# NVIDIA/MinkowskiEngine

Hardware: AMD Instinct MI355X
Metric: MinkowskiConvolution fwd+bwd Mpoints/sec (100k-pt 3D, k=3) (higher is better)
Workload: dtype f32

## Files before the change

minkowskiengine_amd/_lib.py:

```python
import ctypes
import os

_HERE = os.path.dirname(os.path.abspath(__file__))
_TAG = os.environ.get("ME_AMD_LIB_TAG", "")
LIB_PATH = os.path.join(_HERE, f"libme_amd_{_TAG}.so" if _TAG else "libme_amd.so")

ME_MAX_DIM = 7
ME_MAX_TILE_ROWS = 256
ME_GROUP_ROWS = 16
ME_MAX_BATCH_GROUPS = 4

c_i32, c_i64, c_vp = ctypes.c_int32, ctypes.c_int64, ctypes.c_void_p


class MeRegion(ctypes.Structure):
    _fields_ = [
        ("ncol", c_i32),
        ("region_type", c_i32),
        ("kernel_size", c_i32 * ME_MAX_DIM),
        ("dilation", c_i32 * ME_MAX_DIM),
        ("tensor_stride", c_i32 * ME_MAX_DIM),
        ("n_offsets", c_i32),
        ("offsets_dev", c_vp),
    ]
# ... 241 lines not shown
    "me_direct_max_pool_f32": (ctypes.c_int, [c_vp, c_i32, c_vp, c_vp, c_i32, c_i64, c_i64, c_i64, c_i32, c_vp, c_vp, c_vp, c_i64, c_vp]),
    "me_direct_max_pool_bf16": (ctypes.c_int, [c_vp, c_i32, c_vp, c_vp, c_i32, c_i64, c_i64, c_i64, c_i32, c_vp, c_vp, c_vp, c_i64, c_vp]),
    "me_direct_max_pool_f64": (ctypes.c_int, [c_vp, c_i32, c_vp, c_vp, c_i32, c_i64, c_i64, c_i64, c_i32, c_vp, c_vp, c_vp, c_i64, c_vp]),
    "me_direct_max_pool_backward_workspace_bytes": (c_i64, [c_i64, c_i32]),
    "me_direct_max_pool_backward_f32": (ctypes.c_int, [c_vp, c_vp, c_i32, c_i64, c_i32, c_i64, c_vp, c_vp, c_i64, c_vp]),
    "me_direct_max_pool_backward_bf16": (ctypes.c_int, [c_vp, c_vp, c_i32, c_i64, c_i32, c_i64, c_vp, c_vp, c_i64, c_vp]),
    "me_direct_max_pool_backward_f64": (ctypes.c_int, [c_vp, c_vp, c_i32, c_i64, c_i32, c_i64, c_vp, c_vp, c_i64, c_vp]),
    "me_union_tables": (ctypes.c_int, [c_vp, c_i64, c_vp, c_i64, c_i64, c_vp, c_vp, c_vp, c_vp, c_vp]),
    "me_union_arith_f32": (ctypes.c_int, [c_vp, c_vp, c_i32, c_vp, c_vp, c_i64, c_i64, c_i64, c_i32, c_vp, c_vp]),
    "me_union_arith_bf16": (ctypes.c_int, [c_vp, c_vp, c_i32, c_vp, c_vp, c_i64, c_i64, c_i64, c_i32, c_vp, c_vp]),
    "me_union_arith_f64": (ctypes.c_int, [c_vp, c_vp, c_i32, c_vp, c_vp, c_i64, c_i64, c_i64, c_i32, c_vp, c_vp]),
    "me_union_arith_backward_f32": (ctypes.c_int, [c_vp, c_vp, c_vp, c_i32, c_vp, c_vp, c_vp, c_vp, c_i64, c_i64, c_i64, c_i32, c_vp, c_vp, c_vp]),
    "me_union_arith_backward_bf16": (ctypes.c_int, [c_vp, c_vp, c_vp, c_i32, c_vp, c_vp, c_vp, c_vp, c_i64, c_i64, c_i64, c_i32, c_vp, c_vp, c_vp]),
    "me_union_arith_backward_f64": (ctypes.c_int, [c_vp, c_vp, c_vp, c_i32, c_vp, c_vp, c_vp, c_vp, c_i64, c_i64, c_i64, c_i32, c_vp, c_vp, c_vp]),
    "me_csr_from_coo_workspace_bytes": (c_i64, [c_i64]),
    "me_csr_from_coo": (ctypes.c_int, [c_vp, c_vp, c_vp, c_i32, c_i64, c_i64, c_vp, c_vp, c_vp, c_vp, c_i64, c_vp]),
    "me_csr_gather_f32": (ctypes.c_int, [c_vp, c_i32, c_vp, c_vp, c_vp, c_vp, c_i64, c_vp, c_vp]),
    "me_csr_gather_bf16": (ctypes.c_int, [c_vp, c_i32, c_vp, c_vp, c_vp, c_vp, c_i64, c_vp, c_vp]),
    "me_csr_gather_f64": (ctypes.c_int, [c_vp, c_i32, c_vp, c_vp, c_vp, c_vp, c_i64, c_vp, c_vp]),
    "me_conv_forward_naive_f32": (ctypes.c_int, [c_vp, c_i32, c_vp, c_i32, c_vp, c_vp, c_vp, c_i64, c_i64,
                                                 c_vp, c_vp]),
    "me_conv_backward_naive_f32": (ctypes.c_int, [c_vp, c_i32, c_vp, c_i32, c_vp, c_vp, c_vp, c_vp, c_i64,
                                                  c_i64, c_vp, c_vp, c_vp]),
}

DEBUG_SIGNATURES = {
    "me_debug_variants_compiled": (c_i32, []),
    "me_debug_set_conv_variant": (ctypes.c_int, [ctypes.c_int]),
    "me_debug_conv_timing": (ctypes.c_int, [c_vp, c_i32]),
    "me_debug_conv_timing_f32x3": (ctypes.c_int, [c_vp, c_i32]),
    "me_debug_set_wgrad_config": (None, [ctypes.c_int, ctypes.c_int]),
    "me_debug_set_wgrad_order": (None, [ctypes.c_int]),
    "me_debug_set_dgrad_reduce_tail": (None, [ctypes.c_int]),
    "me_debug_set_wgrad_ws": (None, [ctypes.c_int]),
    "me_debug_set_tile_dispatch": (None, [ctypes.c_int]),
    "me_debug_set_wgrad_mb": (None, [ctypes.c_int]),
    "me_debug_set_bf16_shape": (None, [ctypes.c_int, ctypes.c_int]),
    "me_debug_set_bf16_deep": (None, [ctypes.c_int]),
    "me_debug_set_bf16_twobuf": (None, [ctypes.c_int]),
    "me_debug_set_f32_fused_split": (None, [ctypes.c_int]),
    "me_debug_set_bf16_ws": (None, [ctypes.c_int]),
    "me_debug_set_halo": (None, [ctypes.c_int, ctypes.c_int, ctypes.c_int, ctypes.c_int]),
    "me_debug_halo_mode": (c_i32, []),
    "me_debug_set_stem": (None, [ctypes.c_int, ctypes.c_int]),
    "me_debug_set_stem_tiles_per_wg": (None, [ctypes.c_int]),
    "me_debug_halo_timing": (ctypes.c_int, [c_vp, c_i32]),
    "me_debug_set_bf16_ws_fuse": (None, [ctypes.c_int]),
    "me_debug_set_bf16_ws_depth": (None, [ctypes.c_int]),
    "me_debug_set_bf16_ws_ncw": (None, [ctypes.c_int]),
    "me_debug_set_rowwise_groups": (None, [ctypes.c_int]),
    "me_debug_set_rowwise_items_per_wg": (None, [ctypes.c_int]),
    "me_debug_set_insert_fused": (None, [ctypes.c_int]),
    "me_debug_ws_timing": (ctypes.c_int, [c_vp, c_i32]),
    "me_debug_set_bf16_offsync": (None, [ctypes.c_int]),
    "me_debug_set_bf16_splitk": (None, [ctypes.c_int]),
    "me_debug_set_bf16_splitk_mode": (None, [ctypes.c_int]),
    "me_debug_bf16_timing": (ctypes.c_int, [c_vp, c_i32]),
}

_lib = None


def load():
    global _lib
    if _lib is not None:
        return _lib
# ... 72 lines not shown
```

minkowskiengine_amd/csrc/conv_f32x3.hip:

```cpp
#include <type_traits>
#include <vector>
#include "conv_common.hpp"
#include "conv_ws.hpp"
#include "wgrad_reduce.hpp"

namespace me {


__host__ __device__ constexpr int x3_group_shares(int nc) { return nc >= 96 ? 1 : (nc == 64 ? 2 : 4); }

__host__ __device__ constexpr int conv_f32x3_lds_bytes(int nc, int kc, int tile_rows) {
  return (tile_rows + 1) * (nc + kAccPad) * 4 + 2 * ME_MAX_BATCH_GROUPS * 16 * (3 * x3_stage_ld(kc) * 2 + 4);
}

template <int KC>
__global__ __launch_bounds__(256) void k_pack_weights_f32x3(const float *__restrict__ w, int c_src, int c_dst,
                                                           int transposed, int nchunks, int ncb,
                                                           u32x4 *__restrict__ wp, int64_t total) {
  constexpr int KS = KC / 32;
  const int64_t e = (int64_t)blockIdx.x * blockDim.x + threadIdx.x;
  if (e >= total) return;
  const int lane = (int)(e % 64);
  int64_t r = e / 64;
  const int v = (int)(r % KS);
  r /= KS;
  const int cb = (int)(r % ncb);
  r /= ncb;
  const int c = (int)(r % nchunks);
  const int64_t k = r / nchunks;
  const int q = lane >> 4, i16 = lane & 15;
  const int col = cb * 16 + i16;
  float val[8];
#pragma unroll
  for (int j = 0; j < 8; ++j) {
    const int ch = c * KC + v * 32 + q * 8 + j;
    val[j] = 0.f;
    if (ch < c_src && col < c_dst) {
      const int64_t idx = transposed ? (k * c_dst + col) * c_src + ch : (k * c_src + ch) * c_dst + col;
      val[j] = w[idx];
    }
  }
  u32x4 p1, p2, p3;
  split3<true>(f32x4{val[0], val[1], val[2], val[3]}, f32x4{val[4], val[5], val[6], val[7]}, p1, p2, p3);
  const int64_t base = ((((k * nchunks + c) * ncb + cb) * 3) * KS + v) * 64 + lane;
  wp[base] = p1;
// ... 312 lines not shown
#pragma unroll
    for (int j = 0; j < ORD; ++j)
      if (j * NT + tid < tile_rows) s_ord[j * NT + tid] = my_ord[j];
    __syncthreads();
  }
  for (int x = tid; x < tile_rows * NC / 4; x += NT) {
    const int row = x / (NC / 4);
    const int c4 = x % (NC / 4);
    const int cc = col_base + c4 * 4;
    if (row < rows_here && cc < c_dst) {
      const f32x4 v = *reinterpret_cast<const f32x4 *>(&s_acc[row * ACC_LD + c4 * 4]);
      const int64_t grow = order ? (int64_t)s_ord[row] : row0 + row;
      float *o = dst + grow * c_dst + cc;
      if (vec_out) {
        *reinterpret_cast<f32x4 *>(o) = v;
      } else {
        o[0] = v.x;
        if (cc + 1 < c_dst) o[1] = v.y;
        if (cc + 2 < c_dst) o[2] = v.z;
        if (cc + 3 < c_dst) o[3] = v.w;
      }
    }
  }
  if (TIMED) {
    tick(6);
    if (tid == 0) {
#pragma unroll
      for (int t = 0; t < 7; ++t) atomicAdd(&d_x3_timing[t], tm[t]);
      atomicAdd(&d_x3_timing[7], (unsigned long long)n_it);
    }
  }
}

template <typename T>
__device__ __forceinline__ const T &only_arg(const T &t) { return t; }

template <int NC, int KC, bool EXACT, bool SMALL, bool TIMED = false, int PRIO = 2, int ABL = 0, int NCW = 4,
          bool TAIL = false, typename... TAIL_ARG>
__global__ __launch_bounds__((NCW + 4) * 64, 1) void k_conv_tile_f32x3_ws(
    const float *__restrict__ src, int c_src, const bf16x8 *__restrict__ wp, int c_dst,
    const int32_t *__restrict__ plan_src, const int32_t *__restrict__ plan_dst,
    const int32_t *__restrict__ batch_desc, const int32_t *__restrict__ tile_bptr,
    const int32_t *__restrict__ order, float *__restrict__ dst, int64_t n_tgt, int tile_rows, int batch_groups,
    TAIL_ARG... tail) {
  static_assert(sizeof...(TAIL_ARG) == (TAIL ? 1 : 0), "TAIL: exactly one WgTail argument");
  typedef int i32x2 __attribute__((ext_vector_type(2)));
  typedef StageLayout<KC> SL;
  static_assert(NC == 64 || NC == 128, "multiplier waves of 16 or 32 columns");
  static_assert(NCW == 4 || (NCW == 8 && NC == 128), "four multiplier waves, or eight on a 128-column slab");
  constexpr int CB = NC / (16 * NCW);
  constexpr int NTP = 256;
  constexpr int NT = NCW * 64 + NTP;
  constexpr int LD = SL::kLd;
  constexpr int ACC_LD = NC + kAccPad;
  constexpr int KS = KC / 32;
  constexpr int F8 = KC / 8;
  constexpr int CAP = ME_MAX_BATCH_GROUPS * 16;
  constexpr int ITER = (CAP * F8 + NTP - 1) / NTP;
  constexpr int PLANE = CAP * LD;
  (void)batch_groups;

  extern __shared__ __attribute__((aligned(16))) char smem[];
  unsigned n_tiles = gridDim.x;
  if constexpr (TAIL) {
    const WgTail &t = only_arg(tail...);
    n_tiles = (unsigned)t.n_tiles;
    if (blockIdx.x >= n_tiles) {
      if (blockIdx.y + 1 == gridDim.y) wgrad_reduce_tail<NT>(t.r, t.nb, (int)(blockIdx.x - n_tiles), smem);
      return;
    }
  }
  float *s_acc = reinterpret_cast<float *>(smem);
  __bf16 *s_a = reinterpret_cast<__bf16 *>(s_acc + (tile_rows + 1) * ACC_LD);
  int32_t *s_dst = reinterpret_cast<int32_t *>(s_a + 2 * 3 * PLANE);

  const int tid = threadIdx.x;
  const int lane = tid & 63;
  const int wave = __builtin_amdgcn_readfirstlane(tid >> 6);
  const int i16 = lane & 15;
  const int q = lane >> 4;
  const int tile = tile_bptr[n_tiles + 1 + blockIdx.x];
  const int col_base = blockIdx.y * NC;
  const int nchunks = (c_src + KC - 1) / KC;
  const int ncb = (c_dst + 15) / 16;

  for (int x = tid; x < (tile_rows + 1) * ACC_LD / 4; x += NT)
    reinterpret_cast<f32x4 *>(s_acc)[x] = f32x4{0.f, 0.f, 0.f, 0.f};
  constexpr int ORD = (ME_MAX_TILE_ROWS + NT - 1) / NT;
  int32_t my_ord[ORD];
#pragma unroll
  for (int j = 0; j < ORD; ++j) {
    const int r = j * NT + tid;
    my_ord[j] = (order != nullptr && r < tile_rows && (int64_t)tile * tile_rows + r < n_tgt)
                    ? order[(int64_t)tile * tile_rows + r] : 0;
  }

  const int b0 = tile_bptr[tile];
  const int nb = tile_bptr[tile + 1] - b0;
  const int n_it = nb * nchunks;
  struct Desc {
    int chunk, g0, ng, k;
  };
  auto locate = [&](int it) {
    int r = min(it, n_it - 1);
    Desc d;
    d.chunk = 0;
    while (r >= nb) {
      r -= nb;
      ++d.chunk;
    }
    const i32x2 v = *reinterpret_cast<const i32x2 *>(batch_desc + 2 * (int64_t)(b0 + r));
    d.g0 = v.x;
    d.ng = v.y & 255;
    d.k = (int)((uint32_t)v.y >> 8);
    return d;
  };

  if (n_it > 0 && wave >= NCW) {
    const int ptid = tid - NCW * 64;
    f32x4 stage[2][ITER][2];
    int32_t dstv[2] = {tile_rows, tile_rows};
    int32_t sidx[2][ITER];
    auto load_sidx = [&](const Desc &d, int32_t (&sx)[ITER]) {
      const char *pb = reinterpret_cast<const char *>(plan_src + (int64_t)d.g0 * 16);
#pragma unroll
      for (int j = 0; j < ITER; ++j)
        sx[j] = *reinterpret_cast<const int32_t *>(pb + (unsigned)(min((j * NTP + ptid) / F8, CAP - 1) * 4));
    };
    const char *srcb = reinterpret_cast<const char *>(src);
    const unsigned row_bytes = (unsigned)c_src * 4u;
    auto gather = [&](const Desc &d, const int32_t (&sx)[ITER], f32x4 (&st)[ITER][2], int32_t &dv) {
      const int c0 = d.chunk * KC;
      dv = *reinterpret_cast<const int32_t *>(reinterpret_cast<const char *>(plan_dst + (int64_t)d.g0 * 16) +
                                             (unsigned)(min(ptid, CAP - 1) * 4));
#pragma unroll
      for (int j = 0; j < ITER; ++j) {
        const int ch = c0 + ((j * NTP + ptid) % F8) * 8;
        const int chl = EXACT ? ch : min(ch, c_src - 8);
        const int sr = max(sx[j], 0);
        const f32x4 *p;
        if (SMALL) p = reinterpret_cast<const f32x4 *>(srcb + (__umul24((unsigned)sr, row_bytes) + (unsigned)chl * 4u));
        else p = reinterpret_cast<const f32x4 *>(src + (int64_t)sr * c_src + chl);
        st[j][0] = p[0];
        st[j][1] = p[1];
      }
    };
    auto write_stage = [&](const Desc &d, const f32x4 (&st)[ITER][2], int32_t dv, int buf) {
      const int c0 = d.chunk * KC;
// ... 38 lines not shown
    auto produce = [&](const Desc &dx, const Desc &dx2, const Desc &dx3, int buf, f32x4 (&st)[ITER][2], int32_t &dv,
                       int32_t (&sx_nx)[ITER], int32_t (&sx_cu)[ITER]) {
      if (ABL != 6) write_stage(dx, st, dv, buf);
      load_sidx(dx3, sx_cu);
      if (ABL != 5 || !started) gather(dx2, sx_nx, st, dv);
    };
    Desc dA = locate(0), dB = locate(1), dC = locate(2), dD = locate(3), dE = locate(4);
    load_sidx(dA, sidx[0]);
    load_sidx(dB, sidx[1]);
    gather(dA, sidx[0], stage[0], dstv[0]);
    gather(dB, sidx[1], stage[1], dstv[1]);
    load_sidx(dC, sidx[0]);
    produce(dA, dC, dD, 0, stage[0], dstv[0], sidx[0], sidx[1]);
    started = true;
    __syncthreads();
    unsigned long long tm_a = 0, tm_b = 0, t_prev = TIMED ? __builtin_amdgcn_s_memtime() : 0ull;
    auto iteration = [&](int it, int P, f32x4 (&st_nx)[ITER][2], int32_t &dv_nx, int32_t (&sx_nx)[ITER],
                         int32_t (&sx_cu)[ITER]) {
      produce(dB, dD, dE, P ^ 1, st_nx, dv_nx, sx_nx, sx_cu);
      if (TIMED) {
        asm volatile("s_waitcnt lgkmcnt(0)" ::: "memory");
        const unsigned long long now = __builtin_amdgcn_s_memtime();
        tm_a += now - t_prev;
        t_prev = now;
      }
      __syncthreads();
      if (TIMED) {
        const unsigned long long now = __builtin_amdgcn_s_memtime();
        tm_b += now - t_prev;
        t_prev = now;
      }
      dA = dB; dB = dC; dC = dD; dD = dE;
      dE = locate(it + 5);
    };
    int it = 0;
    for (; it + 1 < n_it; it += 2) {
      iteration(it, 0, stage[1], dstv[1], sidx[1], sidx[0]);
      iteration(it + 1, 1, stage[0], dstv[0], sidx[0], sidx[1]);
    }
    if (it < n_it) iteration(it, 0, stage[1], dstv[1], sidx[1], sidx[0]);
    if (TIMED && tid == NCW * 64) {
      atomicAdd(&d_x3_timing[1], tm_a);
      atomicAdd(&d_x3_timing[2], tm_b);
    }
  } else if (n_it > 0) {
    __builtin_amdgcn_s_setprio(PRIO);
    const int cbi0 = col_base / 16 + wave * CB;
    bf16x8 w[2][CB][3][KS];
    auto load_w = [&](const Desc &d, bf16x8 (&wd)[CB][3][KS]) {
#pragma unroll
      for (int c = 0; c < CB; ++c) {
        const bf16x8 *p = wp + (((((int64_t)d.k * nchunks + d.chunk) * ncb + min(cbi0 + c, ncb - 1)) * 3) * KS) * 64 + lane;
#pragma unroll
        for (int pl = 0; pl < 3; ++pl) {
#pragma unroll
          for (int v = 0; v < KS; ++v) wd[c][pl][v] = p[(pl * KS + v) * 64];
        }
      }
    };
    int pofs[KS];
#pragma unroll
    for (int sx = 0; sx < KS; ++sx) pofs[sx] = ((sx * 4 + q) ^ SL::swz(i16)) * 8;
    auto multiply = [&](const Desc &d, const bf16x8 (&wc)[CB][3][KS], int buf, auto &&next_w) {
      const __bf16 *rowp = s_a + buf * 3 * PLANE + i16 * LD;
      const int32_t *dstp = s_dst + buf * CAP + i16;
      float *accp = &s_acc[wave * CB * 16 + q * 4];
      if (d.ng >= 4) consume_batch_ws<2, 2, CB, KC, 3, ABL>(rowp, pofs, wc, dstp, accp, ACC_LD, next_w);
      else if (d.ng == 3) consume_batch_ws<2, 1, CB, KC, 3, ABL>(rowp, pofs, wc, dstp, accp, ACC_LD, next_w);
      else if (d.ng == 2) consume_batch_ws<2, 0, CB, KC, 3, ABL>(rowp, pofs, wc, dstp, accp, ACC_LD, next_w);
      else consume_batch_ws<1, 0, CB, KC, 3, ABL>(rowp, pofs, wc, dstp, accp, ACC_LD, next_w);
    };
    Desc dA = locate(0), dB = locate(1);
    load_w(dA, w[0]);
    __syncthreads();
    unsigned long long tm_a = 0, tm_b = 0, t_prev = TIMED ? __builtin_amdgcn_s_memtime() : 0ull;
    auto iteration = [&](int it, int P, bf16x8 (&w_cu)[CB][3][KS], bf16x8 (&w_nx)[CB][3][KS]) {
      multiply(dA, w_cu, P, [&]() {
        if (ABL != 4 || it == 0) load_w(dB, w_nx);
      });
      if (TIMED) {
        asm volatile("s_waitcnt lgkmcnt(0)" ::: "memory");
        const unsigned long long now = __builtin_amdgcn_s_memtime();
        tm_a += now - t_prev;
        t_prev = now;
      }
      __syncthreads();
      if (TIMED) {
        const unsigned long long now = __builtin_amdgcn_s_memtime();
        tm_b += now - t_prev;
        t_prev = now;
      }
      dA = dB;
      dB = locate(it + 2);
    };
    int it = 0;
    for (; it + 1 < n_it; it += 2) {
      iteration(it, 0, w[0], w[1]);
      iteration(it + 1, 1, w[1], w[0]);
    }
    if (it < n_it) iteration(it, 0, w[0], w[1]);
    if (TIMED && tid == 0) {
      atomicAdd(&d_x3_timing[4], tm_a);
      atomicAdd(&d_x3_timing[0], tm_b);
      atomicAdd(&d_x3_timing[7], (unsigned long long)n_it);
    }
  } else {
    __syncthreads();
  }

  const int64_t row0 = (int64_t)tile * tile_rows;
  const int rows_here = (int)min((int64_t)tile_rows, n_tgt - row0);
  const bool vec_out = (c_dst % 4) == 0;
  int32_t *s_ord = reinterpret_cast<int32_t *>(s_a);
  if (order != nullptr) {
#pragma unroll
    for (int j = 0; j < ORD; ++j)
      if (j * NT + tid < tile_rows) s_ord[j * NT + tid] = my_ord[j];
    __syncthreads();
  }
  for (int x = tid; x < tile_rows * NC / 4; x += NT) {
    const int row = x / (NC / 4);
    const int c4 = x % (NC / 4);
    const int cc = col_base + c4 * 4;
    if (row < rows_here && cc < c_dst) {
      const f32x4 v = *reinterpret_cast<const f32x4 *>(&s_acc[row * ACC_LD + c4 * 4]);
      const int64_t grow = order ? (int64_t)s_ord[row] : row0 + row;
      float *o = dst + grow * c_dst + cc;
      if (vec_out) {
        *reinterpret_cast<f32x4 *>(o) = v;
      } else {
        o[0] = v.x;
        if (cc + 1 < c_dst) o[1] = v.y;
        if (cc + 2 < c_dst) o[2] = v.z;
        if (cc + 3 < c_dst) o[3] = v.w;
      }
    }
  }
}


#ifdef ME_DEBUG_VARIANTS
__device__ __forceinline__ unsigned ring_addr(const int32_t *p) {
  typedef __attribute__((address_space(3))) const char lds_char;
  return (unsigned)(uintptr_t)(lds_char *)p;
}
__device__ __forceinline__ void ring_wait(unsigned flag_addr, int target) {
  for (;;) {
    int v;
    asm volatile("ds_read_b32 %0, %1\n\ts_waitcnt lgkmcnt(0)" : "=v"(v) : "v"(flag_addr) : "memory");
    if (__builtin_amdgcn_readfirstlane(v) >= target) break;
    __builtin_amdgcn_s_sleep(1);
  }
}
__device__ __forceinline__ void ring_signal(unsigned flag_addr, int lane) {
  if (lane == 0) asm volatile("ds_add_u32 %0, %1" : : "v"(flag_addr), "v"(1) : "memory");
}

__host__ __device__ constexpr int conv_f32x3_ring_lds_bytes(int nc, int kc, int tile_rows, int ns) {
  return (tile_rows + 1) * (nc + kAccPad) * 4 + ns * ME_MAX_BATCH_GROUPS * 16 * (3 * x3_stage_ld(kc) * 2 + 4) + 64;
}

template <int NC, int KC, bool EXACT, bool SMALL, int NCW, int NS>
__global__ __launch_bounds__((NCW + 4) * 64, 1) void k_conv_tile_f32x3_ring(
    const float *__restrict__ src, int c_src, const bf16x8 *__restrict__ wp, int c_dst,
    const int32_t *__restrict__ plan_src, const int32_t *__restrict__ plan_dst,
    const int32_t *__restrict__ batch_desc, const int32_t *__restrict__ tile_bptr,
    const int32_t *__restrict__ order, float *__restrict__ dst, int64_t n_tgt, int tile_rows, int batch_groups) {
  typedef int i32x2 __attribute__((ext_vector_type(2)));
  typedef StageLayout<KC> SL;
// ... 578 lines not shown
        ++round;
      }
    };
    for (;;) {
      iteration(w[0], w[1]);
      if (end) break;
      iteration(w[1], w[0]);
      if (end) break;
    }
  }
}

#endif

extern int g_conv_variant;

struct ConvVariantX3 {
  int nc, slabs, kc;
};

static ConvVariantX3 conv_variant_f32x3(int c_src, int c_dst) {
  ConvVariantX3 v;
  if (c_dst % 128 == 0) v.nc = 128;
  else if (c_dst % 96 == 0) v.nc = 96;
  else v.nc = c_dst <= 32 ? 32 : 64;
  v.slabs = (int)ceil_div(c_dst, v.nc);
  if (c_src % 128 == 0 && v.nc <= 64) v.kc = 128;
  else if (c_src % 64 == 0) v.kc = 64;
  else if (c_src % 96 == 0) v.kc = 96;
  else v.kc = c_src <= 32 ? 32 : 64;
  return v;
}

template <int NC, int KC>
static int launch_conv_tile_f32x3(const float *src, int c_src, const bf16x8 *wp, int c_dst, int slabs,
                                  const int32_t *plan_src, const int32_t *plan_dst, const int32_t *batch_desc,
                                  const int32_t *tile_bptr, const int32_t *order, float *dst, int64_t n_tgt,
                                  int tile_rows, int batch_groups, hipStream_t stream, bool small,
                                  const WgTail *tail = nullptr) {
  int lds = conv_f32x3_lds_bytes(NC, KC, tile_rows);
  ME_CHECK(lds <= kLdsBudget, "tile_rows too large for the LDS of one workgroup");
  const bool exact = (c_src % KC) == 0;
  const bool fast = small && exact;
  typedef void (*kernel_t)(const float *, int, const bf16x8 *, int, const int32_t *, const int32_t *, const int32_t *,
                           const int32_t *, const int32_t *, float *, int64_t, int, int);
#ifdef ME_DEBUG_VARIANTS
  constexpr bool kHasPingPong = true;
#else
  constexpr bool kHasPingPong = !(NC == 64 || NC == 128);
#endif
  kernel_t fn = nullptr;
  if constexpr (kHasPingPong)
    fn = fast ? &k_conv_tile_f32x3<NC, KC, true, true> : &k_conv_tile_f32x3<NC, KC, false, false>;
  if constexpr (NC == 64 || NC == 128) {
#ifdef ME_DEBUG_VARIANTS
    if constexpr (KC == 64 || KC == 128) {
      if (small && exact && (g_conv_variant == 40 || g_conv_variant == 41)) {
        constexpr int RNCW = NC == 128 ? 8 : 4;
        constexpr bool kHas3 = KC == 64;
        const bool three = kHas3 && g_conv_variant != 41 && conv_f32x3_ring_lds_bytes(NC, KC, tile_rows, 3) <= kLdsBudget;
        kernel_t rk = &k_conv_tile_f32x3_ring<NC, KC, true, true, RNCW, 2>;
        if constexpr (kHas3) {
          if (three) rk = &k_conv_tile_f32x3_ring<NC, KC, true, true, RNCW, 3>;
        }
        const int rlds = conv_f32x3_ring_lds_bytes(NC, KC, tile_rows, three ? 3 : 2);
        ME_CHECK(rlds <= kLdsBudget, "tile_rows too large for the LDS of one workgroup (ring kernel)");
        static bool ring_attr[2] = {false, false};
        if (rlds > 48 * 1024 && !ring_attr[three ? 1 : 0]) {
          ME_HIP(hipFuncSetAttribute(reinterpret_cast<const void *>(rk), hipFuncAttributeMaxDynamicSharedMemorySize,
                                     kLdsBudget));
          ring_attr[three ? 1 : 0] = true;
        }
        const dim3 rgrid((unsigned)ceil_div(n_tgt, tile_rows), (unsigned)slabs);
        hipLaunchKernelGGL(rk, rgrid, dim3((RNCW + 4) * 64), (size_t)rlds, stream, src, c_src, wp, c_dst, plan_src, plan_dst,
// ... 14 lines not shown
        if (plds > 48 * 1024 && !pers_attr) {
          ME_HIP(hipFuncSetAttribute(reinterpret_cast<const void *>(pk), hipFuncAttributeMaxDynamicSharedMemorySize,
                                     kLdsBudget));
          pers_attr = true;
        }
        const int n_tiles = pers_tiles, wgs = pers_wgs;
        hipLaunchKernelGGL(pk, dim3((unsigned)wgs, (unsigned)slabs), dim3((RNCW + 4) * 64), (size_t)plds, stream, src, c_src,
                           wp, c_dst, plan_src, plan_dst, batch_desc, tile_bptr, order, dst, n_tgt, tile_rows, n_tiles);
        ME_LAUNCH_CHECK();
        return 0;
      }
    }
#endif
    if (tail != nullptr) {
      typedef void (*tail_kernel_t)(const float *, int, const bf16x8 *, int, const int32_t *, const int32_t *,
                                    const int32_t *, const int32_t *, const int32_t *, float *, int64_t, int, int, WgTail);
      constexpr int TNCW = NC == 128 ? 8 : 4;
      constexpr int TNT = (TNCW + 4) * 64;
      const tail_kernel_t tk = fast ? &k_conv_tile_f32x3_ws<NC, KC, true, true, false, 2, 0, TNCW, true, WgTail>
                                    : &k_conv_tile_f32x3_ws<NC, KC, false, false, false, 2, 0, TNCW, true, WgTail>;
      const int tail_lds = (TNT / kWgReduceGroup) * kWgReduceGroupLds;
      if (lds < tail_lds) lds = tail_lds;
      static bool tail_attr[2] = {false, false};
      if (lds > 48 * 1024 && !tail_attr[fast ? 1 : 0]) {
        ME_HIP(hipFuncSetAttribute(reinterpret_cast<const void *>(tk), hipFuncAttributeMaxDynamicSharedMemorySize,
                                   kLdsBudget));
        tail_attr[fast ? 1 : 0] = true;
      }
      WgTail t = *tail;
      const int64_t n_tiles = ceil_div(n_tgt, tile_rows);
      const int64_t n_tail = ceil_div(wgrad_tail_groups(t), (int64_t)(TNT / kWgReduceGroup));
      ME_CHECK(n_tiles + n_tail < (1ll << 31), "grid too large");
      t.n_tiles = (int)n_tiles;
      hipLaunchKernelGGL(tk, dim3((unsigned)(n_tiles + n_tail), (unsigned)slabs), dim3(TNT), (size_t)lds, stream, src,
                         c_src, wp, c_dst, plan_src, plan_dst, batch_desc, tile_bptr, order, dst, n_tgt, tile_rows,
                         batch_groups, t);
      ME_LAUNCH_CHECK();
      return 0;
    }
    if (!kHasPingPong || (g_conv_variant != 30 && g_conv_variant != 256)) {
      kernel_t ws;
      int wi = (small ? 2 : 0) + (exact ? 1 : 0);
      int wthreads = 512;
      static bool ws_attr[20] = {};
      if constexpr (NC == 128) {
#ifdef ME_DEBUG_VARIANTS
        if (g_conv_variant == 31) {
          ws = fast ? &k_conv_tile_f32x3_ws<NC, KC, true, true> : &k_conv_tile_f32x3_ws<NC, KC, false, false>;
        } else
#endif
        {
          ws = fast ? &k_conv_tile_f32x3_ws<NC, KC, true, true, false, 2, 0, 8>
                    : &k_conv_tile_f32x3_ws<NC, KC, false, false, false, 2, 0, 8>;
          wi += 13;
          wthreads = 768;
        }
      } else {
        ws = fast ? &k_conv_tile_f32x3_ws<NC, KC, true, true> : &k_conv_tile_f32x3_ws<NC, KC, false, false>;
      }
#ifdef ME_DEBUG_VARIANTS
      if constexpr (KC >= 64) {
        if (g_conv_variant == 257 && small && exact) {
          ws = &k_conv_tile_f32x3_ws<NC, KC, true, true, true>;
          wi = 4;
          wthreads = 512;
        }
        if (g_conv_variant == 32 && small && exact) {
          ws = &k_conv_tile_f32x3_ws<NC, KC, true, true, false, 0>;
          wi = 5;
          wthreads = 512;
// ... 156 lines not shown
#undef ME_CONV_CASE
}

int me_conv_target_f32x3(const float *src, int64_t n_src, int32_t c_src, const uint16_t *wp_, int64_t volume,
                         int32_t c_dst, const int32_t *plan_src, const int32_t *plan_dst, const int32_t *batch_desc,
                         const int32_t *tile_bptr, const int32_t *order, float *dst, int64_t n_tgt, int32_t tile_rows,
                         int32_t batch_groups, void *stream_) {
  (void)volume;
  return conv_target_f32x3(src, n_src, c_src, wp_, c_dst, plan_src, plan_dst, batch_desc, tile_bptr, order, dst, n_tgt,
                           tile_rows, batch_groups, (hipStream_t)stream_, nullptr);
}

int g_dgrad_tail = 0;

constexpr int kTailMaxRounds = 5;

int32_t me_conv_dgrad_reduce_tail_supported(int32_t c_in, int32_t c_out, int64_t volume, int64_t n_pairs) {
  if (g_dgrad_tail == 1 || volume < 1 || volume > 65535 || (g_conv_variant != 0 && g_conv_variant != 6)) return 0;
  if (!me_conv_f32x3_supported(c_out, c_in)) return 0;
  const ConvVariantX3 v = conv_variant_f32x3(c_out, c_in);
  if (v.nc != 64 && v.nc != 128) return 0;
  std::vector<int64_t> koffs((size_t)volume + 1, 0);
  koffs[(size_t)volume] = n_pairs;
  WgTail t;
  if (!wgrad_split_tail(koffs.data(), nullptr, volume, c_in, c_out, nullptr, nullptr, &t)) return 0;
  if (g_dgrad_tail == 2) return 1;
  if (v.slabs != 1) return 0;
  const int groups_per_wg = v.nc == 128 ? 3 : 2;
  return ceil_div(wgrad_tail_groups(t), (int64_t)groups_per_wg) <= (int64_t)kTailMaxRounds * device_cu_count() ? 1 : 0;
}

void me_debug_set_dgrad_reduce_tail(int mode) { g_dgrad_tail = mode; }

int me_conv_dgrad_reduce_tail_f32x3(const float *dy, int64_t n_out, int32_t c_out, const uint16_t *wp_, int64_t volume,
                                    int32_t c_in, const int32_t *plan_src, const int32_t *plan_dst,
                                    const int32_t *batch_desc, const int32_t *tile_bptr, const int32_t *order, float *dx,
                                    int64_t n_in, int32_t tile_rows, int32_t batch_groups, const int64_t *k_offsets,
                                    const int64_t *k_offsets_dev, const void *workspace, int64_t workspace_bytes,
                                    float *grad_w, void *stream_) {
  ME_CHECK(n_in > 0, "no input rows: nothing carries the tail (me_conv_wgrad_f32 handles empty maps)");
  ME_CHECK(g_conv_variant == 0 || g_conv_variant == 6, "debug kernel variants have no reduce tail");
  ME_CHECK(k_offsets != nullptr && k_offsets_dev != nullptr && workspace != nullptr && grad_w != nullptr,
           "pair offsets, workspace and grad_w must not be null");
  ME_CHECK(workspace_bytes >= me_conv_wgrad_workspace_bytes(k_offsets, volume, c_in, c_out), "workspace too small");
  WgTail t;
  ME_CHECK(wgrad_split_tail(k_offsets, k_offsets_dev, volume, c_in, c_out, workspace, grad_w, &t),
           "not a split weight gradient (me_conv_dgrad_reduce_tail_supported)");
  return conv_target_f32x3(dy, n_out, c_out, wp_, c_in, plan_src, plan_dst, batch_desc, tile_bptr, order, dx, n_in,
                           tile_rows, batch_groups, (hipStream_t)stream_, &t);
}

}

extern "C" __attribute__((visibility("hidden"))) void me_preload_conv_f32x3(void) {
  hipFuncAttributes attr;
  (void)hipFuncGetAttributes(&attr, reinterpret_cast<const void *>(&me::k_pack_weights_f32x3<128>));
}
```

minkowskiengine_amd/csrc/me_amd_debug.h:

```cpp
#ifndef ME_AMD_DEBUG_H
#define ME_AMD_DEBUG_H
#include <stdint.h>
#ifdef __cplusplus
extern "C" {
#endif
#if defined(__GNUC__) || defined(__clang__)
#pragma GCC visibility push(default)
#endif

int32_t me_debug_variants_compiled(void);
int me_debug_set_conv_variant(int variant);
int me_debug_conv_timing(uint64_t *out8, int32_t reset);
int me_debug_conv_timing_f32x3(uint64_t *out8, int32_t reset);
void me_debug_set_bf16_shape(int nc, int kc);
void me_debug_set_bf16_deep(int deep);
void me_debug_set_bf16_twobuf(int mode);
void me_debug_set_f32_fused_split(int mode);
void me_debug_set_bf16_ws(int mode);
void me_debug_set_bf16_ws_fuse(int mode);
void me_debug_set_bf16_ws_depth(int depth);
void me_debug_set_bf16_ws_ncw(int ncw);
int me_debug_ws_timing(uint64_t *out8, int32_t reset);
void me_debug_set_bf16_offsync(int mode);
void me_debug_set_bf16_splitk(int g);
void me_debug_set_bf16_splitk_mode(int same_tiles);
int me_debug_bf16_timing(uint64_t *out20, int32_t reset);
void me_debug_set_wgrad_config(int depth, int wgs_per_cu);
void me_debug_set_wgrad_order(int mode);
void me_debug_set_dgrad_reduce_tail(int mode);
void me_debug_set_tile_dispatch(int mode);
void me_debug_set_wgrad_mb(int mb);
void me_debug_set_wgrad_ws(int mode);

void me_debug_set_halo(int mode, int tile_rows, int kc, int skip);
int32_t me_debug_halo_mode(void);
int me_debug_halo_timing(uint64_t *out8, int32_t reset);
void me_debug_set_stem(int mode, int groups);
void me_debug_set_stem_tiles_per_wg(int tiles);
void me_debug_set_insert_fused(int on);
void me_debug_set_rowwise_groups(int groups);
void me_debug_set_rowwise_items_per_wg(int items);

#if defined(__GNUC__) || defined(__clang__)
#pragma GCC visibility pop
#endif
#ifdef __cplusplus
}
#endif
#endif
```

Baseline: 340.8.

## Chain multiple output tiles per persistent workgroup in f32x3 conv kernel

Adds a persistent 'tile chain' mode: instead of one workgroup per output tile, launches one workgroup per CU slot, and each walks a serpentine-assigned list of tiles. The producer/consumer pipeline keeps running across tile boundaries and flushes the accumulator between tiles, so per-tile launch, prologue and pipeline-drain costs go away and load across CUs is balanced. It is enabled by default when tiles outnumber CUs. It adds LDS for the chain table and row order, plus extra syncs at each tile rollover, and it also adds some timing instrumentation.

New measurement: 343.6, median of 6. About the same (+0.8%).

```diff
diff --git a/minkowskiengine_amd/_lib.py b/minkowskiengine_amd/_lib.py
--- a/minkowskiengine_amd/_lib.py
+++ b/minkowskiengine_amd/_lib.py
@@ -297,6 +297,9 @@
     "me_debug_set_wgrad_config": (None, [ctypes.c_int, ctypes.c_int]),
     "me_debug_set_wgrad_order": (None, [ctypes.c_int]),
     "me_debug_set_dgrad_reduce_tail": (None, [ctypes.c_int]),
+    "me_debug_set_tile_chain": (None, [ctypes.c_int]),
+    "me_debug_set_tile_chain_slots": (None, [ctypes.c_int]),
+    "me_debug_last_tile_chain": (c_i32, []),
     "me_debug_set_wgrad_ws": (None, [ctypes.c_int]),
     "me_debug_set_tile_dispatch": (None, [ctypes.c_int]),
     "me_debug_set_wgrad_mb": (None, [ctypes.c_int]),
diff --git a/minkowskiengine_amd/csrc/conv_f32x3.hip b/minkowskiengine_amd/csrc/conv_f32x3.hip
--- a/minkowskiengine_amd/csrc/conv_f32x3.hip
+++ b/minkowskiengine_amd/csrc/conv_f32x3.hip
@@ -9,8 +9,15 @@
 
 __host__ __device__ constexpr int x3_group_shares(int nc) { return nc >= 96 ? 1 : (nc == 64 ? 2 : 4); }
 
-__host__ __device__ constexpr int conv_f32x3_lds_bytes(int nc, int kc, int tile_rows) {
-  return (tile_rows + 1) * (nc + kAccPad) * 4 + 2 * ME_MAX_BATCH_GROUPS * 16 * (3 * x3_stage_ld(kc) * 2 + 4);
+struct TileChain {
+  int n_tiles;
+  int slots;
+};
+constexpr int kChainMaxTiles = 32;
+
+__host__ __device__ constexpr int conv_f32x3_lds_bytes(int nc, int kc, int tile_rows, bool chain = false) {
+  return (tile_rows + 1) * (nc + kAccPad) * 4 + 2 * ME_MAX_BATCH_GROUPS * 16 * (3 * x3_stage_ld(kc) * 2 + 4) +
+         (chain ? kChainMaxTiles * 16 + (tile_rows + 1) * 4 : 0);
 }
 
 template <int KC>
@@ -389,8 +396,12 @@
   }
 }
 
+template <typename T, typename... R>
+__device__ __forceinline__ const T &first_arg(const T &t, const R &...) { return t; }
 template <typename T>
-__device__ __forceinline__ const T &only_arg(const T &t) { return t; }
+__device__ __forceinline__ const T &last_arg(const T &t) { return t; }
+template <typename T, typename U, typename... R>
+__device__ __forceinline__ const auto &last_arg(const T &, const U &u, const R &... r) { return last_arg(u, r...); }
 
 template <int NC, int KC, bool EXACT, bool SMALL, bool TIMED = false, int PRIO = 2, int ABL = 0, int NCW = 4,
           bool TAIL = false, typename... TAIL_ARG>
@@ -400,8 +411,11 @@
     const int32_t *__restrict__ batch_desc, const int32_t *__restrict__ tile_bptr,
     const int32_t *__restrict__ order, float *__restrict__ dst, int64_t n_tgt, int tile_rows, int batch_groups,
     TAIL_ARG... tail) {
-  static_assert(sizeof...(TAIL_ARG) == (TAIL ? 1 : 0), "TAIL: exactly one WgTail argument");
+  constexpr bool CHAIN = (std::is_same<TAIL_ARG, TileChain>::value || ...);
+  static_assert(sizeof...(TAIL_ARG) == (TAIL ? 1 : 0) + (CHAIN ? 1 : 0), "TAIL: one WgTail argument; CHAIN: one TileChain behind it");
+  static_assert(!CHAIN || (!TIMED && ABL == 0), "no instrumented chain kernel");
   typedef int i32x2 __attribute__((ext_vector_type(2)));
+  typedef int i32x4 __attribute__((ext_vector_type(4)));
   typedef StageLayout<KC> SL;
   static_assert(NC == 64 || NC == 128, "multiplier waves of 16 or 32 columns");
   static_assert(NCW == 4 || (NCW == 8 && NC == 128), "four multiplier waves, or eight on a 128-column slab");
@@ -419,24 +433,35 @@
 
   extern __shared__ __attribute__((aligned(16))) char smem[];
   unsigned n_tiles = gridDim.x;
+  unsigned slots = 0;
+  if constexpr (CHAIN) {
+    const TileChain &c = last_arg(tail...);
+    n_tiles = (unsigned)c.n_tiles;
+    slots = (unsigned)c.slots;
+  }
   if constexpr (TAIL) {
-    const WgTail &t = only_arg(tail...);
-    n_tiles = (unsigned)t.n_tiles;
-    if (blockIdx.x >= n_tiles) {
-      if (blockIdx.y + 1 == gridDim.y) wgrad_reduce_tail<NT>(t.r, t.nb, (int)(blockIdx.x - n_tiles), smem);
+    const WgTail &t = first_arg(tail...);
+    if constexpr (!CHAIN) n_tiles = (unsigned)t.n_tiles;
+    const unsigned n_front = CHAIN ? slots : n_tiles;
+    if (blockIdx.x >= n_front) {
+      if (blockIdx.y + 1 == gridDim.y) wgrad_reduce_tail<NT>(t.r, t.nb, (int)(blockIdx.x - n_front), smem);
       return;
     }
   }
   float *s_acc = reinterpret_cast<float *>(smem);
   __bf16 *s_a = reinterpret_cast<__bf16 *>(s_acc + (tile_rows + 1) * ACC_LD);
   int32_t *s_dst = reinterpret_cast<int32_t *>(s_a + 2 * 3 * PLANE);
+  int32_t *s_chain = s_dst + 2 * CAP;
+  int32_t *s_rows = s_chain + 4 * kChainMaxTiles;
 
   const int tid = threadIdx.x;
   const int lane = tid & 63;
   const int wave = __builtin_amdgcn_readfirstlane(tid >> 6);
   const int i16 = lane & 15;
   const int q = lane >> 4;
-  const int tile = tile_bptr[n_tiles + 1 + blockIdx.x];
+  const unsigned long long t_enter = TIMED ? __builtin_amdgcn_s_memtime() : 0ull;
+  unsigned long long t_tail = 0;
+  const int tile = CHAIN ? 0 : tile_bptr[n_tiles + 1 + blockIdx.x];
   const int col_base = blockIdx.y * NC;
   const int nchunks = (c_src + KC - 1) / KC;
   const int ncb = (c_dst + 15) / 16;
@@ -445,32 +470,147 @@
     reinterpret_cast<f32x4 *>(s_acc)[x] = f32x4{0.f, 0.f, 0.f, 0.f};
   constexpr int ORD = (ME_MAX_TILE_ROWS + NT - 1) / NT;
   int32_t my_ord[ORD];
-#pragma unroll
-  for (int j = 0; j < ORD; ++j) {
-    const int r = j * NT + tid;
-    my_ord[j] = (order != nullptr && r < tile_rows && (int64_t)tile * tile_rows + r < n_tgt)
-                    ? order[(int64_t)tile * tile_rows + r] : 0;
-  }
-
-  const int b0 = tile_bptr[tile];
-  const int nb = tile_bptr[tile + 1] - b0;
-  const int n_it = nb * nchunks;
+  if constexpr (!CHAIN) {
+#pragma unroll
+    for (int j = 0; j < ORD; ++j) {
+      const int r = j * NT + tid;
+      my_ord[j] = (order != nullptr && r < tile_rows && (int64_t)tile * tile_rows + r < n_tgt)
+                      ? order[(int64_t)tile * tile_rows + r] : 0;
+    }
+  }
+  auto load_ord = [&](int tl) {
+#pragma unroll
+    for (int j = 0; j < ORD; ++j) {
+      const int r = j * NT + tid;
+      my_ord[j] = (order != nullptr && r < tile_rows && (int64_t)tl * tile_rows + r < n_tgt)
+                      ? order[(int64_t)tl * tile_rows + r] : 0;
+    }
+  };
+
+  int n_chain = 0;
+  int chain_its = 0;
+  auto chain_entry = [&](int k, int &tl, int &first, int &count) {
+    const i32x4 v = reinterpret_cast<const i32x4 *>(s_chain)[k];
+    tl = __builtin_amdgcn_readfirstlane(v.x);
+    first = __builtin_amdgcn_readfirstlane(v.y);
+    count = __builtin_amdgcn_readfirstlane(v.z);
+  };
+  if constexpr (CHAIN) {
+    const unsigned g = blockIdx.x, G = slots;
+    const unsigned rem = n_tiles % (2 * G);
+    n_chain = (int)(2 * (n_tiles / (2 * G)) + (rem > g ? 1 : 0) + (rem > 2 * G - 1 - g ? 1 : 0));
+    if (tid < n_chain) {
+      const unsigned pos = (tid & 1) ? (unsigned)(tid + 1) * G - 1 - g : (unsigned)tid * G + g;
+      const int tl = tile_bptr[n_tiles + 1 + pos];
+      const int first = tile_bptr[tl];
+      reinterpret_cast<i32x4 *>(s_chain)[tid] = i32x4{tl, first, tile_bptr[tl + 1] - first, 0};
+    }
+    __syncthreads();
+    for (int k = 0; k < n_chain; ++k) {
+      int tl, first, count;
+      chain_entry(k, tl, first, count);
+      chain_its += count * nchunks;
+    }
+  }
+  int e_k = 0, e_end = 0;
+  auto roll_as = [&](auto ordered) {
+    constexpr bool ORDERED = decltype(ordered)::value;
+    for (;;) {
+      int tl, first, count;
+      chain_entry(e_k, tl, first, count);
+      if constexpr (ORDERED) {
+#pragma unroll
+        for (int j = 0; j < ORD; ++j)
+          if (j * NT + tid < tile_rows) s_rows[j * NT + tid] = my_ord[j];
+        __syncthreads();
+      }
+      const int64_t row0 = (int64_t)tl * tile_rows;
+      const int rows_here = (int)min((int64_t)tile_rows, n_tgt - row0);
+      const bool vec_out = (c_dst % 4) == 0;
+      for (int x = tid; x < (tile_rows + 1) * (NC / 4); x += NT) {
+        const int row = x / (NC / 4);
+        const int c4 = x % (NC / 4);
+        const int cc = col_base + c4 * 4;
+        f32x4 *a = reinterpret_cast<f32x4 *>(&s_acc[row * ACC_LD + c4 * 4]);
+        const f32x4 v = *a;
+        *a = f32x4{0.f, 0.f, 0.f, 0.f};
+        if (row < rows_here && cc < c_dst) {
+          const int64_t grow = ORDERED ? (int64_t)s_rows[row] : row0 + row;
+          float *o = dst + grow * c_dst + cc;
+          if (vec_out) {
+            *reinterpret_cast<f32x4 *>(o) = v;
+          } else {
+            o[0] = v.x;
+            if (cc + 1 < c_dst) o[1] = v.y;
+            if (cc + 2 < c_dst) o[2] = v.z;
+            if (cc + 3 < c_dst) o[3] = v.w;
+          }
+        }
+      }
+      count = 0;
+      if (++e_k < n_chain) {
+        chain_entry(e_k, tl, first, count);
+        if constexpr (ORDERED) load_ord(tl);
+      }
+      __syncthreads();
+      if (e_k >= n_chain || count > 0) {
+        e_end += count * nchunks;
+        break;
+      }
+    }
+  };
+  auto roll = [&]() {
+    if (order != nullptr) roll_as(std::true_type{});
+    else roll_as(std::false_type{});
+  };
+  if constexpr (CHAIN) {
+    int tl, first, count;
+    chain_entry(0, tl, first, count);
+    if (order != nullptr) load_ord(tl);
+    if (count > 0) e_end = count * nchunks;
+    else roll();
+  }
+
+  const int b0 = CHAIN ? 0 : tile_bptr[tile];
+  const int nb = CHAIN ? 0 : tile_bptr[tile + 1] - b0;
+  const int n_it = CHAIN ? chain_its : nb * nchunks;
   struct Desc {
     int chunk, g0, ng, k;
   };
+  int c_k = -1, c_b0 = 0, c_nb = 1, c_base = 0, c_end = 0;
   auto locate = [&](int it) {
     int r = min(it, n_it - 1);
     Desc d;
     d.chunk = 0;
-    while (r >= nb) {
-      r -= nb;
-      ++d.chunk;
-    }
-    const i32x2 v = *reinterpret_cast<const i32x2 *>(batch_desc + 2 * (int64_t)(b0 + r));
-    d.g0 = v.x;
-    d.ng = v.y & 255;
-    d.k = (int)((uint32_t)v.y >> 8);
-    return d;
+    if constexpr (CHAIN) {
+      while (r >= c_end) {
+        int tl;
+        do chain_entry(++c_k, tl, c_b0, c_nb);
+        while (c_nb == 0);
+        c_base = c_end;
+        c_end += c_nb * nchunks;
+      }
+      r -= c_base;
+      while (r >= c_nb) {
+        r -= c_nb;
+        ++d.chunk;
+      }
+      const i32x2 v = *reinterpret_cast<const i32x2 *>(batch_desc + 2 * (int64_t)(c_b0 + r));
+      d.g0 = v.x;
+      d.ng = v.y & 255;
+      d.k = (int)((uint32_t)v.y >> 8);
+      return d;
+    } else {
+      while (r >= nb) {
+        r -= nb;
+        ++d.chunk;
+      }
+      const i32x2 v = *reinterpret_cast<const i32x2 *>(batch_desc + 2 * (int64_t)(b0 + r));
+      d.g0 = v.x;
+      d.ng = v.y & 255;
+      d.k = (int)((uint32_t)v.y >> 8);
+      return d;
+    }
   };
 
   if (n_it > 0 && wave >= NCW) {
@@ -575,6 +715,9 @@
       }
       dA = dB; dB = dC; dC = dD; dD = dE;
       dE = locate(it + 5);
+      if constexpr (CHAIN) {
+        if (it + 1 == e_end) roll();
+      }
     };
     int it = 0;
     for (; it + 1 < n_it; it += 2) {
@@ -617,6 +760,7 @@
     load_w(dA, w[0]);
     __syncthreads();
     unsigned long long tm_a = 0, tm_b = 0, t_prev = TIMED ? __builtin_amdgcn_s_memtime() : 0ull;
+    if (TIMED && tid == 0) atomicAdd(&d_x3_timing[5], t_prev - t_enter);
     auto iteration = [&](int it, int P, bf16x8 (&w_cu)[CB][3][KS], bf16x8 (&w_nx)[CB][3][KS]) {
       multiply(dA, w_cu, P, [&]() {
         if (ABL != 4 || it == 0) load_w(dB, w_nx);
@@ -635,6 +779,9 @@
       }
       dA = dB;
       dB = locate(it + 2);
+      if constexpr (CHAIN) {
+        if (it + 1 == e_end) roll();
+      }
     };
     int it = 0;
     for (; it + 1 < n_it; it += 2) {
@@ -646,10 +793,12 @@
       atomicAdd(&d_x3_timing[4], tm_a);
       atomicAdd(&d_x3_timing[0], tm_b);
       atomicAdd(&d_x3_timing[7], (unsigned long long)n_it);
+      t_tail = t_prev;
     }
   } else {
-    __syncthreads();
-  }
+    if constexpr (!CHAIN) __syncthreads();
+  }
+  if constexpr (CHAIN) return;
 
   const int64_t row0 = (int64_t)tile * tile_rows;
   const int rows_here = (int)min((int64_t)tile_rows, n_tgt - row0);
@@ -678,6 +827,12 @@
         if (cc + 3 < c_dst) o[3] = v.w;
       }
     }
+  }
+  if (TIMED && tid == 0 && n_it > 0) {
+    const unsigned long long t_issued = __builtin_amdgcn_s_memtime();
+    asm volatile("s_waitcnt vmcnt(0)" ::: "memory");
+    atomicAdd(&d_x3_timing[6], t_issued - t_tail);
+    atomicAdd(&d_x3_timing[3], __builtin_amdgcn_s_memtime() - t_tail);
   }
 }
 
@@ -1322,6 +1477,23 @@
   return v;
 }
 
+int g_tile_chain = 0;
+int g_tile_chain_slots = 0;
+int g_last_tile_chain = 0;
+
+template <int NC, int KC>
+constexpr bool kHasTileChain = (NC == 64 || NC == 128) && !(NC == 128 && KC == 96);
+
+template <int NC, int KC>
+static int tile_chain_slots(int64_t n_tiles, int tile_rows) {
+  if (!kHasTileChain<NC, KC> || g_tile_chain == 1 || (g_conv_variant != 0 && g_conv_variant != 6)) return 0;
+  int64_t G = g_tile_chain_slots > 0 ? g_tile_chain_slots : device_cu_count();
+  if (g_tile_chain == 0 && n_tiles <= G) return 0;
+  if (G > n_tiles) G = n_tiles;
+  if (ceil_div(n_tiles, G) > kChainMaxTiles || conv_f32x3_lds_bytes(NC, KC, tile_rows, true) > kLdsBudget) return 0;
+  return (int)G;
+}
+
 template <int NC, int KC>
 static int launch_conv_tile_f32x3(const float *src, int c_src, const bf16x8 *wp, int c_dst, int slabs,
                                   const int32_t *plan_src, const int32_t *plan_dst, const int32_t *batch_desc,
@@ -1330,6 +1502,7 @@
                                   const WgTail *tail = nullptr) {
   int lds = conv_f32x3_lds_bytes(NC, KC, tile_rows);
   ME_CHECK(lds <= kLdsBudget, "tile_rows too large for the LDS of one workgroup");
+  g_last_tile_chain = 0;
   const bool exact = (c_src % KC) == 0;
   const bool fast = small && exact;
   typedef void (*kernel_t)(const float *, int, const bf16x8 *, int, const int32_t *, const int32_t *, const int32_t *,
@@ -1410,10 +1583,52 @@
       const int64_t n_tail = ceil_div(wgrad_tail_groups(t), (int64_t)(TNT / kWgReduceGroup));
       ME_CHECK(n_tiles + n_tail < (1ll << 31), "grid too large");
       t.n_tiles = (int)n_tiles;
+      if constexpr (kHasTileChain<NC, KC>) if (const int G = tile_chain_slots<NC, KC>(n_tiles, tile_rows)) {
+        typedef void (*chain_kernel_t)(const float *, int, const bf16x8 *, int, const int32_t *, const int32_t *,
+                                       const int32_t *, const int32_t *, const int32_t *, float *, int64_t, int, int, WgTail,
+                                       TileChain);
+        const chain_kernel_t ck = fast ? &k_conv_tile_f32x3_ws<NC, KC, true, true, false, 2, 0, TNCW, true, WgTail, TileChain>
+                                       : &k_conv_tile_f32x3_ws<NC, KC, false, false, false, 2, 0, TNCW, true, WgTail, TileChain>;
+        int clds = conv_f32x3_lds_bytes(NC, KC, tile_rows, true);
+        if (clds < tail_lds) clds = tail_lds;
+        static bool chain_attr[2] = {false, false};
+        if (clds > 48 * 1024 && !chain_attr[fast ? 1 : 0]) {
+          ME_HIP(hipFuncSetAttribute(reinterpret_cast<const void *>(ck), hipFuncAttributeMaxDynamicSharedMemorySize,
+                                     kLdsBudget));
+          chain_attr[fast ? 1 : 0] = true;
+        }
+        const TileChain c{(int)n_tiles, G};
+        hipLaunchKernelGGL(ck, dim3((unsigned)(G + n_tail), (unsigned)slabs), dim3(TNT), (size_t)clds, stream, src, c_src,
+                           wp, c_dst, plan_src, plan_dst, batch_desc, tile_bptr, order, dst, n_tgt, tile_rows,
+                           batch_groups, t, c);
+        ME_LAUNCH_CHECK();
+        g_last_tile_chain = G;
+        return 0;
+      }
       hipLaunchKernelGGL(tk, dim3((unsigned)(n_tiles + n_tail), (unsigned)slabs), dim3(TNT), (size_t)lds, stream, src,
                          c_src, wp, c_dst, plan_src, plan_dst, batch_desc, tile_bptr, order, dst, n_tgt, tile_rows,
                          batch_groups, t);
       ME_LAUNCH_CHECK();
+      return 0;
+    }
+    if constexpr (kHasTileChain<NC, KC>) if (const int G = tile_chain_slots<NC, KC>(ceil_div(n_tgt, tile_rows), tile_rows)) {
+      typedef void (*chain_kernel_t)(const float *, int, const bf16x8 *, int, const int32_t *, const int32_t *,
+                                     const int32_t *, const int32_t *, const int32_t *, float *, int64_t, int, int, TileChain);
+      constexpr int CNCW = NC == 128 ? 8 : 4;
+      const chain_kernel_t ck = fast ? &k_conv_tile_f32x3_ws<NC, KC, true, true, false, 2, 0, CNCW, false, TileChain>
+                                     : &k_conv_tile_f32x3_ws<NC, KC, false, false, false, 2, 0, CNCW, false, TileChain>;
+      const int clds = conv_f32x3_lds_bytes(NC, KC, tile_rows, true);
+      static bool chain_attr[2] = {false, false};
+      if (clds > 48 * 1024 && !chain_attr[fast ? 1 : 0]) {
+        ME_HIP(hipFuncSetAttribute(reinterpret_cast<const void *>(ck), hipFuncAttributeMaxDynamicSharedMemorySize,
+                                   kLdsBudget));
+        chain_attr[fast ? 1 : 0] = true;
+      }
+      const TileChain c{(int)ceil_div(n_tgt, tile_rows), G};
+      hipLaunchKernelGGL(ck, dim3((unsigned)G, (unsigned)slabs), dim3((CNCW + 4) * 64), (size_t)clds, stream, src, c_src, wp,
+                         c_dst, plan_src, plan_dst, batch_desc, tile_bptr, order, dst, n_tgt, tile_rows, batch_groups, c);
+      ME_LAUNCH_CHECK();
+      g_last_tile_chain = G;
       return 0;
     }
     if (!kHasPingPong || (g_conv_variant != 30 && g_conv_variant != 256)) {
@@ -1636,6 +1851,13 @@
 
 void me_debug_set_dgrad_reduce_tail(int mode) { g_dgrad_tail = mode; }
 
+void me_debug_set_tile_chain(int mode) {
+  g_tile_chain = mode;
+  g_last_tile_chain = -1;
+}
+void me_debug_set_tile_chain_slots(int g) { g_tile_chain_slots = g > 0 ? g : 0; }
+int32_t me_debug_last_tile_chain(void) { return g_last_tile_chain; }
+
 int me_conv_dgrad_reduce_tail_f32x3(const float *dy, int64_t n_out, int32_t c_out, const uint16_t *wp_, int64_t volume,
                                     int32_t c_in, const int32_t *plan_src, const int32_t *plan_dst,
                                     const int32_t *batch_desc, const int32_t *tile_bptr, const int32_t *order, float *dx,
diff --git a/minkowskiengine_amd/csrc/me_amd_debug.h b/minkowskiengine_amd/csrc/me_amd_debug.h
--- a/minkowskiengine_amd/csrc/me_amd_debug.h
+++ b/minkowskiengine_amd/csrc/me_amd_debug.h
@@ -28,6 +28,9 @@
 void me_debug_set_wgrad_config(int depth, int wgs_per_cu);
 void me_debug_set_wgrad_order(int mode);
 void me_debug_set_dgrad_reduce_tail(int mode);
+void me_debug_set_tile_chain(int mode);
+void me_debug_set_tile_chain_slots(int g);
+int32_t me_debug_last_tile_chain(void);
 void me_debug_set_tile_dispatch(int mode);
 void me_debug_set_wgrad_mb(int mb);
 void me_debug_set_wgrad_ws(int mode);
```
